# better-flow/better-flow

Hardware: AMD Instinct MI355X
Metric: Mevents/s motion-compensated (warp→converged score), 1M-ev slice, 1/2/4/8 GPU (higher is better)
Workload: dtype f64

## Files before the change

### better_flow_amd/csrc/bf_context.cpp

```cpp
#include "bf_ctx.h"

std::atomic<int> g_live_ctx[64];

extern "C" {

const char* bf_version(void) { return "bf_accel gfx950 r5"; }

int bf_device_count(int32_t* count) {
    int n = 0;
    hipError_t e = hipGetDeviceCount(&n);
    if (count) *count = (e == hipSuccess) ? n : 0;
    return (e == hipSuccess && n > 0) ? BF_OK : BF_ERR_NODEVICE;
}

int bf_abi_struct_sizes(int32_t* out, int32_t n) {
    const int32_t sz[10] = {(int32_t)sizeof(bf_model),     (int32_t)sizeof(bf_window),
                            (int32_t)sizeof(bf_run_opts),  (int32_t)sizeof(bf_run_info),
                            (int32_t)sizeof(bf_trace_rec), (int32_t)sizeof(bf_profile),
                            (int32_t)sizeof(bf_local_window), (int32_t)sizeof(bf_local_state),
                            (int32_t)sizeof(bf_global_pyramid_opts), (int32_t)sizeof(bf_global_pyramid_info)};
    if (!out) return 10;
    const int32_t m = n < 0 ? 0 : (n < 10 ? n : 10);
    for (int i = 0; i < m; ++i) out[i] = sz[i];
    return m;
// ... 140 lines not shown
    }
    delete c;
}

const char* bf_last_error(const bf_ctx* c) {
    if (!c) return "null ctx";
    static thread_local char text[sizeof(c->err)];
    std::lock_guard<std::mutex> g(const_cast<bf_ctx*>(c)->err_mu);
    memcpy(text, c->err, sizeof(text));
    text[sizeof(text) - 1] = 0;
    return text;
}

int bf_get_stat(bf_ctx* c, const char* key, int64_t* value) {
    if (!c || !key || !value) return BF_ERR_ARG;
    if (!strcmp(key, "scatter_format")) {
        *value = c->use_binned ? c->fmt : -1;
        return BF_OK;
    }
    if (!strcmp(key, "one_kernel")) {
        *value = plan_one_kernel(c) ? 1 : 0;
        return BF_OK;
    }
    if (!strcmp(key, "persistent")) {
        *value = plan_persistent(c) ? 1 : 0;
        return BF_OK;
    }
    if (!strcmp(key, "persist_giveups")) {
        *value = c->persist_giveups;
        return BF_OK;
    }
    const struct { const char* name; int v; } launched[] = {
        {"k1_threads", c->launched.k1_threads}, {"k1_events_per_thread", c->launched.k1_per_thread}, {"k1_head", c->launched.k1_head},
        {"k3_half_scale", c->launched.k3_half_scale}, {"k3_mode", c->launched.k3_mode}, {"k3_capped", c->launched.k3_capped},
        {"bin_rows", c->use_binned ? c->grid.TSR : 0}, {"bin_cols", c->use_binned ? c->grid.TS : 0},
        {"bin_margin", c->use_binned ? c->grid.D : 0}, {"bins", c->use_binned ? c->grid.nbins : 0},
        {"groups_lds", c->groups_lds}, {"groups_per_cu", c->groups_per_cu},
        {"propose_form", c->propose_form}};
    for (const auto& e : launched)
        if (!strcmp(key, e.name)) {
            *value = e.v;
            return BF_OK;
        }
    return fail(c, BF_ERR_ARG, "unknown statistic '%s'", key);
}

int bf_set_option(bf_ctx* c, const char* key, int64_t value) {
    if (!c || !key) return BF_ERR_ARG;
    if (!strcmp(key, "force_split")) {
        c->force_split = value != 0;
        return BF_OK;
    }
    if (!strcmp(key, "binned")) {
        if (value < 0 || value > 2) return fail(c, BF_ERR_ARG, "binned must be 0, 1 or 2");
        c->opt_binned = (int)value;
        return BF_OK;
    }
    if (!strcmp(key, "bin_pack_limit")) {
        if (value < 1 || value > 64) return fail(c, BF_ERR_ARG, "bin_pack_limit must be in [1, 64]");
        c->opt_bin_pack_limit = (int)value;
        return BF_OK;
    }
    if (!strcmp(key, "co_schedule")) {
        c->opt_co_schedule = value != 0;
        return BF_OK;
    }
    if (!strcmp(key, "stream_prealloc")) {
        if (!value) return BF_OK;
        HIP_TRY(c, hipSetDevice(c->device));
        const int rc = streaming_setup(c);
        if (rc != BF_OK) return rc;
        for (bf_ctx::UploadSlot& s : c->up.slot) {
            HIP_TRY(c, s.ts.grow((size_t)c->cap_events));
            HIP_TRY(c, s.in16.grow((size_t)c->cap_events * 2));
            HIP_TRY(c, s.noise.grow((size_t)c->cap_events));
        }
        return BF_OK;
    }
    if (!strcmp(key, "sep_update")) {
        if (value < 0 || value > 2) return fail(c, BF_ERR_ARG, "sep_update must be 0 (never), 1 (auto) or 2 (always)");
        c->opt_sep_update = (int)value;
        return BF_OK;
    }
    if (!strcmp(key, "defer_uploads")) {
        if (!value) {
            HIP_TRY(c, hipSetDevice(c->device));
            const int rc = issue_deferred_uploads(c);
            if (rc != BF_OK) return rc;
        }
        c->opt_defer_uploads = value != 0;
        return BF_OK;
    }
    if (!strcmp(key, "watchdog_ms")) {
        if (value < 1) return fail(c, BF_ERR_ARG, "watchdog_ms must be >= 1");
        c->opt_watchdog_s = (double)value * 1e-3;
        return BF_OK;
    }
    if (!strcmp(key, "bin_compact")) {
        if (value < 0 || value > 2) return fail(c, BF_ERR_ARG, "bin_compact must be 0 (never), 1 (auto) or 2 (always)");
        c->opt_bin_compact = (int)value;
        return BF_OK;
    }
    if (!strcmp(key, "bin_split")) {
        if (value < 0 || value > 2) return fail(c, BF_ERR_ARG, "bin_split must be 0, 1 or 2");
        c->opt_bin_split = (int)value;
        return BF_OK;
    }
    if (!strcmp(key, "bin_predict")) {
        c->opt_bin_predict = value != 0;
        return BF_OK;
    }
    if (!strcmp(key, "fused")) {
        if (value < 0 || value > 2) return fail(c, BF_ERR_ARG, "fused must be 0, 1 (auto) or 2");
// ... 188 lines not shown
```

### better_flow_amd/csrc/bf_ctx.h

```cpp
#pragma once
#pragma clang diagnostic ignored "-Wunused-function"
#include <hip/hip_runtime.h>

#include <atomic>
#include <cerrno>
#include <climits>
#include <cmath>
#include <cstdarg>
#include <cstdio>
#include <cstdlib>
#include <chrono>
#include <cstring>
#include <ctime>
#include <memory>
#include <mutex>
#include <new>
#include <utility>
#include <string>
#include <thread>
#include <vector>

#include "bf_assign.h"
#include "bf_device.h"
#include "bf_kernels.h"
// ... 174 lines not shown
    DevArray<uint8_t> d_seg_mask;
    bool seg_valid = false;
    int seg_K = 0;
    SliceStats stats;
    bool stats_valid = false;

    HostArray<DevState> h_state;
    unsigned long long* h_seq = nullptr;
    unsigned long long seq_counter = 0;
    Event poll_ev[2];
    double opt_watchdog_s = 40.0;
    HostArray<SliceStats> h_stats;

    DevState hst;
    bf_window win;
    bool uploaded = false, have_window = false;
    bool has_noise = false, all_noise = false;
    bool packed = true;
    bool force_split = false;
    bool degenerate = false;
    bool pending_warp = false;
    bool n_valid = false;
    uint32_t run_counter = 0;
    int warm_iters_hint = 6;
    bool p_clean = false;
    bool out_sorted = false;
    DevArray<double2> d_out_tmp;
    bool uv_valid = false;
    int cur = 0;
    bool planes_unknown = true;
    int last_R = 0, last_C = 0;

    struct Launched {
        int k1_threads = -1, k1_per_thread = -1, k1_head = -1;
        int k3_half_scale = -1, k3_mode = -1, k3_capped = -1;
    } launched;

    int prof_mode = 0;
    std::vector<ProfRec> prof_pending;
    std::vector<Event> ev_pool;
    bf_profile prof;

    char err[512];
    std::mutex err_mu;
};

extern "C" int ctx_device_uv(bf_ctx* c, const double2** uv);

extern "C" int ctx_device_nxny(bf_ctx* c, const double2** nxny);

struct GlobalHeldFlow {
    const uint32_t* xy; const float2* p; const uint32_t* idx; const double2 *nxny, *uv;
    long long n;
};
int global_held_flow(bf_ctx* c, const char* who, GlobalHeldFlow* out);

struct GlobalBestState {
    const double *max_score, *best_nx, *best_ny;
    long long n;
    double nz;
};
int global_best_state(bf_ctx* c, const bf_global_search_opts* lattice, std::vector<double>& xs, std::vector<double>& ys,
                      GlobalBestState* out);
void global_cand_uv(double nx, double ny, double nz, double* u, double* v);

extern "C" int render_projection_img(bf_ctx* c, int32_t scale, int32_t res_x, int32_t res_y, int32_t show_final, uint8_t* d_img);
extern "C" int render_projection_img_of(bf_ctx* c, const uint32_t* xy, const float2* p, const uint8_t* noise, long long n,
                                        int32_t scale, int32_t res_x, int32_t res_y, int32_t show_final, uint8_t* d_img);
extern "C" int render_color_time_img(bf_ctx* c, int32_t scale, int32_t res_x, int32_t res_y, int32_t show_final, uint8_t* d_bgr);

int ctx_time_img_pass(bf_ctx* c, const char* who);

struct SlicePlan {
    BinGrid grid{}, fgrid{};
    bool binned = false, fused_ok = false, fused_shared = false;
    int fmt = 0, zw = 0;
};
struct RunPlan {
    bool fused = false, binned = false, persist = false;
    bool head_update = false, sep_update = false;
    bool split = false;
    int bin_threads = 0, ev_per_thread = 8;
    bool warm_start = false, prewarp = false, first_warp = false;
    bool quick_warm = false, snap_polled = false;
    double drift_limit = 1e300;
    bool head_like() const { return head_update || sep_update; }
};
SlicePlan plan_slice(const bf_ctx* c, const bf_window& w);
bool plan_one_kernel(const bf_ctx* c);
bool plan_persistent(const bf_ctx* c);
RunPlan plan_run(bf_ctx* c, const bf_run_opts& o);

int streaming_setup(bf_ctx* c);
int issue_deferred_uploads(bf_ctx* c);
void drop_uploads(bf_ctx* c, int k);

namespace {

int fail(bf_ctx* c, int code, const char* fmt, ...) {
    if (c) {
        va_list ap;
        va_start(ap, fmt);
        std::lock_guard<std::mutex> g(c->err_mu);
        vsnprintf(c->err, sizeof(c->err), fmt, ap);
        va_end(ap);
    }
    return code;
}

#define HIP_TRY(c, expr)                                                                      \
    do {                                                                                      \
        hipError_t e__ = (expr);                                                              \
        if (e__ != hipSuccess)                                                                \
            return fail((c), BF_ERR_HIP, "%s failed: %s (%s:%d)", #expr, hipGetErrorString(e__), \
                        __FILE__, __LINE__);                                                  \
    } while (0)

Event get_event(bf_ctx* c) {
    Event e;
// ... 328 lines not shown
```

### better_flow_amd/csrc/bf_device_fns.h

```cpp
#pragma once
#include <hip/hip_runtime.h>
#include <limits.h>

#include "bf_device.h"
#include "bf_kernels.h"
#include "../../include/bf_flow_color.h"
#include <math.h>
#include <math.h>

namespace bf {

__device__ __forceinline__ int trunc_x86(double v) { return bf_double_to_int_x86(v); }

__device__ __forceinline__ int trunc_scatter(double v) { return (v == v) ? __double2int_rz(v) : INT_MIN; }

__device__ __forceinline__ bool valid_px(float p) { return p > 1e-6f; }

__device__ __forceinline__ double div_10000(double x) {
    constexpr double R = 1.0 / 10000.0;
    const double q0 = x * R;
    const double r = fma(-q0, 10000.0, x);
    return fma(r, R, q0);
}
__device__ __forceinline__ float div_127(float x) {
// ... 265 lines not shown
    for (int w = 0; w < W; ++w) {
#pragma unroll
        for (int f = 0; f < 3; ++f) in_[f] += (long long)s_part[f * W + w];
#pragma unroll
        for (int f = 3; f < kSumFields; ++f) d_[f - 3] += __longlong_as_double((long long)s_part[f * W + w]);
    }
    t.n = in_[0]; t.sci = in_[1]; t.scj = in_[2];
    t.sgx = d_[0]; t.sgy = d_[1]; t.sigx = d_[2]; t.sigy = d_[3]; t.sjgx = d_[4]; t.sjgy = d_[5];
    return t;
}
template <int THREADS, bool PACK_INTS = false>
__device__ __forceinline__ Sums block_reduce_sums(const Sums& sm, unsigned long long* s_part ,
                                                  const int tid, const int base_i = 0, const int base_j = 0) {
    block_reduce_publish<THREADS, PACK_INTS>(sm, s_part, tid, base_i, base_j);
    return block_reduce_total<THREADS, PACK_INTS>(s_part, base_i, base_j);
}

struct RcpTab {
    double v[kRcpTab];
    constexpr RcpTab() : v{} {
        for (int i = 1; i < kRcpTab; ++i) v[i] = 1.0 / (double)i;
    }
};
static __constant__ RcpTab c_rcp = RcpTab();

__device__ __forceinline__ float time_from_sums(uint32_t cnt, long long tsum_biased, long long tmin, const double* rcp = nullptr) {
    if (cnt == 0) return 0.f;
    const long long ts = tsum_biased + (long long)(int)cnt * (long long)(int)tmin;
    const float sum_s = (float)div_1e9((double)ts);
    if (rcp && cnt < (uint32_t)kRcpTab) return (float)((double)sum_s * rcp[cnt]);
    return sum_s / (float)cnt;
}

__device__ __attribute__((noinline)) static void sincos_large(double x, double* sn, double* cs) { sincos(x, sn, cs); }
__device__ __forceinline__ void sincos_small(double x, double* sn, double* cs) {
    if (!(fabs(x) <= 0.25)) {
        sincos_large(x, sn, cs);
        return;
    }
    const double z = x * x;
    double ps = -1.0 / 1307674368000.0;
    ps = fma(ps, z, 1.0 / 6227020800.0);
    ps = fma(ps, z, -1.0 / 39916800.0);
    ps = fma(ps, z, 1.0 / 362880.0);
    ps = fma(ps, z, -1.0 / 5040.0);
    ps = fma(ps, z, 1.0 / 120.0);
    ps = fma(ps, z, -1.0 / 6.0);
    *sn = fma(x * z, ps, x);
    double pc = 1.0 / 20922789888000.0;
    pc = fma(pc, z, -1.0 / 87178291200.0);
    pc = fma(pc, z, 1.0 / 479001600.0);
    pc = fma(pc, z, -1.0 / 3628800.0);
    pc = fma(pc, z, 1.0 / 40320.0);
    pc = fma(pc, z, -1.0 / 720.0);
    pc = fma(pc, z, 1.0 / 24.0);
    *cs = 1.0 - z * fma(-z, pc, 0.5);
}

__device__ __forceinline__ void sincos_table_fill(double* tab) {
    tab[0] = -1.0 / 1307674368000.0; tab[1] = 1.0 / 6227020800.0; tab[2] = -1.0 / 39916800.0; tab[3] = 1.0 / 362880.0;
    tab[4] = -1.0 / 5040.0; tab[5] = 1.0 / 120.0; tab[6] = -1.0 / 6.0;
    tab[7] = 1.0 / 20922789888000.0; tab[8] = -1.0 / 87178291200.0; tab[9] = 1.0 / 479001600.0; tab[10] = -1.0 / 3628800.0;
    tab[11] = 1.0 / 40320.0; tab[12] = -1.0 / 720.0; tab[13] = 1.0 / 24.0;
}
__device__ __forceinline__ void sincos_small_tab(double x, const double* tab, double* sn, double* cs) {
    if (!(fabs(x) <= 0.25)) {
        sincos_large(x, sn, cs);
        return;
    }
    const double z = x * x;
    double c_[14];
#pragma unroll
    for (int i = 0; i < 14; ++i) c_[i] = tab[i];
    double ps = c_[0];
    ps = fma(ps, z, c_[1]);
    ps = fma(ps, z, c_[2]);
    ps = fma(ps, z, c_[3]);
    ps = fma(ps, z, c_[4]);
    ps = fma(ps, z, c_[5]);
    ps = fma(ps, z, c_[6]);
    *sn = fma(x * z, ps, x);
    double pc = c_[7];
    pc = fma(pc, z, c_[8]);
    pc = fma(pc, z, c_[9]);
    pc = fma(pc, z, c_[10]);
    pc = fma(pc, z, c_[11]);
    pc = fma(pc, z, c_[12]);
    pc = fma(pc, z, c_[13]);
    *cs = 1.0 - z * fma(-z, pc, 0.5);
}

__device__ __forceinline__ double lane_f64(double v, int lane) {
    const long long b = __double_as_longlong(v);
    const unsigned int lo = (unsigned int)__builtin_amdgcn_readlane((int)(unsigned int)b, lane);
    const unsigned int hi = (unsigned int)__builtin_amdgcn_readlane((int)(unsigned int)((unsigned long long)b >> 32), lane);
    return __longlong_as_double((long long)(((unsigned long long)hi << 32) | (unsigned long long)lo));
}
__device__ __forceinline__ long long lane_i64(unsigned long long v, int lane) {
    const unsigned int lo = (unsigned int)__builtin_amdgcn_readlane((int)(unsigned int)v, lane);
    const unsigned int hi = (unsigned int)__builtin_amdgcn_readlane((int)(unsigned int)(v >> 32), lane);
// ... 396 lines not shown
```

### better_flow_amd/csrc/bf_kernels.h

```cpp
#pragma once
#include <hip/hip_runtime.h>
#include <hip/hip_ext.h>
#include <stdint.h>
#include <atomic>

#include "bf_device.h"
#include "bf_plan_rules.h"

namespace bf {

constexpr int kHistCopies = 8;
using bf_rules::kBinTileLdsMax;
static_assert(bf_rules::kStencilTileR == kTileR && bf_rules::kStencilTileC == kTileC, "the rules count the stencil kernel's own tiles");
constexpr int kPrepBlocks = 1024;

struct SliceStats {
    int32_t xmin, xmax, ymin, ymax, tmin, tmax;
    long long tsum;
};

struct WarpScatterArgs {
    const uint32_t* xy;
    const int32_t* t;
    float2* p;
// ... 126 lines not shown
void launch_fill_states(DevState* states, const DevState& tmpl, int nt, hipStream_t s);
constexpr int kGroupLdsBudget = 156 * 1024;
int launch_group_sort(const uint32_t* xy, const int32_t* t, const uint32_t* perm_in, long long n, const int32_t* gid, int K,
                      uint32_t* hist, uint32_t* start, uint32_t* cursor, uint32_t* oxy, int32_t* ot, float2* op,
                      uint32_t* operm, hipStream_t s);
void launch_group_boxes(const uint32_t* xy, const uint32_t* perm, const int32_t* gid, const uint32_t* start, long long n, int K,
                        int32_t* box, hipStream_t s);
int launch_group_optimizer(const TileArgs& a, const uint32_t* order, int K, bool warm, uint32_t* counter, int n_cus,
                           hipStream_t s, int* per_cu_out);
void launch_group_rest(const uint32_t* perm, const uint32_t* start, int K, double2* nxny, hipStream_t s);

int bin_kernel_setup();
void launch_stencil_binned(const StencilArgs& a, dim3 grid, hipStream_t s, int n_cus);
void launch_margin_clean(unsigned long long* mplane, const uint32_t* mlist, uint32_t* mcount, int nbins, int mcap, hipStream_t s);
void launch_rebin(const EvSets& sets, int has_perm, long long n, DevState* st, const BinGrid& g,
                  uint16_t* binid, uint32_t* hist_cnt, uint32_t* bin_start,
                  uint32_t* cursor, uint32_t* armed, const WarpParams* prewarp, int pack_limit, hipStream_t s,
                  uint32_t* ftab = nullptr, uint32_t* lost = nullptr);
struct BinScatterArgs {
    EvSets sets;
    const uint32_t* bin_start;
    unsigned long long* slabs;
    uint16_t* cidx;
    uint32_t* chdr;
    int compact;
    unsigned long long* ovf_plane;
    uint32_t* ovf_cplane;
    uint32_t* ovf_bits;
    int ovf_pitch;
    const DevState* st_in;
    DevState* st_out;
    DevState* snap;
    MomentAcc* acc;
    uint32_t* ovf_cur;
    const uint32_t* ovf_prev;
    bf_trace_rec* trace;
    BinGrid g;
    int cur, j;
    unsigned long long* tl;
    unsigned long long* m_cur;
    unsigned long long* m_prev;
    uint32_t* mlist;
    uint32_t* mcount;
    int mcap;
};
hipError_t launch_bin_warp_scatter(const BinScatterArgs& a, bool warp, int threads, int per_thread, hipStream_t s);
struct FusedArgs {
    EvSets sets;
    const uint32_t* ftab;
    const DevState* st_in;
    DevState* st_out;
    DevState* snap;
    MomentAcc* acc_in;
    MomentAcc* acc_out;
    MomentAcc* acc_zero;
    uint32_t* lost;
    bf_trace_rec* trace;
    int nbr, nbc;
    int R, C;
    int j;
    int warp;
    unsigned long long* tl;
};
hipError_t launch_fused_pass(const FusedArgs& a, int half_scale, int rows_per_tile, hipStream_t s);
struct FusedLoopArgs {
    EvSets sets;
// ... 188 lines not shown
```

### better_flow_amd/csrc/bf_plan.cpp

```cpp
#include "bf_ctx.h"

SlicePlan plan_slice(const bf_ctx* c, const bf_window& w) {
    SlicePlan p;
    const int scale = w.scale;
    BinGrid& g = p.grid;
    const int bin_margin = bf_rules::bin_margin(c->dbg_margin);
    const bf_rules::BinShape shape = bf_rules::bin_shape(c->n, w.scale_img_x, w.scale_img_y, c->n_cus, bin_margin);
    g.TS = shape.TS;
    g.TSR = shape.TSR;
    g.lg = 0;
    while ((1 << g.lg) < g.TS) ++g.lg;
    g.nbc = shape.nbc;
    g.D = shape.D;
    g.L = g.TS + 2 * g.D;
    g.LR = g.TSR + 2 * g.D;
    g.mul_r = (uint32_t)(0x100000000ull / (unsigned)g.TSR) + 1u;
    g.mul_l = (uint32_t)(0x100000000ull / (unsigned)g.L) + 1u;
    g.mul_h = (uint32_t)(0x100000000ull / (unsigned)(g.L / 2 > 0 ? g.L / 2 : 1)) + 1u;
    g.nbr = shape.nbr;
    g.nbins = shape.nbins;
    const bool dense = (double)w.scale_img_x * (double)w.scale_img_y < 12.0 * (double)c->n ||
                       (double)w.scale_img_x * (double)w.scale_img_y <= 9.0e6;
    p.binned = (c->opt_binned == 2 || (c->opt_binned == 1 && dense)) && !c->force_split && !c->has_noise && c->n > 0 &&
               c->cap_events < (1ll << 29) &&
// ... 23 lines not shown
    const bool lists_ok = p.binned && bf_rules::bin_format_ok(shape, 2);
    const int mode = lists_ok ? c->opt_bin_compact : 0;
    if (mode == 2 || (mode == 1 && 4.0 * (double)c->n < Pimg)) p.fmt = 2;
    const bool split_pays = !c->opt_co_schedule && Pimg >= 1.5e6;
    if (p.fmt == 0 && p.binned && (c->opt_bin_split == 2 || (c->opt_bin_split == 1 && split_pays)) &&
        bf_rules::bin_format_ok(shape, 3))
        p.fmt = 3;
    if (p.fmt == 2 && g.TS == 64 && g.L >= 2 * (g.D + scale / 2 + 1)) p.zw = g.D + scale / 2 + 1;
    return p;
}

bool plan_one_kernel(const bf_ctx* c) {
    return c->fused_ok && (!c->opt_co_schedule || c->fused_shared);
}

bool plan_persistent(const bf_ctx* c) {
    return plan_one_kernel(c) && !c->opt_co_schedule && (c->opt_persist == 2 || (c->opt_persist == 1 && c->pending_warp)) &&
           g_live_ctx[c->device & 63].load() == 1 &&
           fused_loop_resident(c->win.scale / 2, c->fgrid.TSR, c->n_cus, c->fgrid.nbr * c->fgrid.nbc);
}

RunPlan plan_run(bf_ctx* c, const bf_run_opts& o) {
    RunPlan p;
    p.fused = plan_one_kernel(c);
    p.binned = c->use_binned || p.fused;
    p.persist = plan_persistent(c);
    if (p.persist && c->persist_skip > 0) { --c->persist_skip; p.persist = false; }
    p.warm_start = c->pending_warp;
    p.prewarp = p.binned && c->pending_warp;
    p.first_warp = c->pending_warp && !p.prewarp;
    if (p.binned) p.drift_limit = c->opt_bin_predict ? (p.persist ? 0.85 : 0.6) * (double)(p.fused ? c->fgrid.D : c->grid.D) : 1e300;
    p.split = c->use_binned && !p.fused && c->fmt == 3;
    p.head_update = p.fused || (p.binned && !c->opt_co_schedule);
    p.sep_update = p.binned && !p.fused && !p.head_update && (c->opt_sep_update == 2 || (c->opt_sep_update == 1 && c->fmt == 2));
    if (p.binned) {
        const bf_rules::ScatterSize k1 = bf_rules::scatter_size(c->fmt, p.head_update, c->grid.nbins, c->n, c->n_cus);
        p.bin_threads = k1.threads;
        p.ev_per_thread = k1.per_thread;
    }
    p.quick_warm = p.warm_start && c->warm_iters_hint < 3 * o.poll_interval;
    p.snap_polled = p.binned && !p.quick_warm;
    return p;
}
```

### better_flow_amd/csrc/bf_run.cpp

```cpp
#include "bf_ctx.h"

namespace {

struct HostTiming {
#ifdef BF_DEBUG_HOOKS
    bool on = [] { static const bool e = getenv("BF_HOST_TIMING") != nullptr; return e; }();
#else
    static constexpr bool on = false;
#endif
    double launch = 0, wait = 0, mark = on ? now() : 0;
    static double now() { return std::chrono::duration<double>(std::chrono::steady_clock::now().time_since_epoch()).count(); }
    void lap(double& into) { if (on) { const double t = now(); into += t - mark; mark = t; } }
};

struct RunLoop {
    bf_ctx* c;
    const RunPlan& p;
    int b0 = 0, buf = 0;
    bool first = true;
    int launched_iters = 0;
    bool prewarp_done = false;
    bf_trace_rec* trace = nullptr;
    bool want_rebin = false;
    int last_rebin_at = 0;
// ... 155 lines not shown
        FusedArgs fa;
        fa.sets = ev_sets(c);
        fa.ftab = c->d_ftab;
        fa.st_in = L.state_of(j); fa.st_out = L.state_of(j + 1);
        fa.snap = snap;
        fa.acc_in = L.acc_of(j - 1); fa.acc_out = L.acc_of(j); fa.acc_zero = L.acc_of(j + 1);
        fa.lost = lost_flag(c);
        fa.trace = L.trace;
        fa.nbr = c->fgrid.nbr; fa.nbc = c->fgrid.nbc;
        fa.R = c->win.scale_img_x; fa.C = c->win.scale_img_y;
        fa.j = j;
        fa.warp = warp ? 1 : 0;
        fa.tl = c->d_tl;
        ProfScope ps(c, 0, c->n);
        HIP_TRY(c, launch_fused_pass(fa, c->win.scale / 2, c->fgrid.TSR, c->stream));
        L.inf.launches += 1;
    } else {
        const int buf = L.buf;
        if (p.sep_update) {
            launch_finish_update(L.state_of(j), L.acc_of(j - 1), L.ovf_of(j - 1), j, buf ^ 1, L.trace, snap, c->stream);
            L.inf.launches++;
        }
        if (p.binned) {
            BinScatterArgs ba;
            ba.sets = ev_sets(c);
            ba.bin_start = c->d_bin_start;
            ba.slabs = c->d_slabs;
            ba.cidx = c->d_cidx; ba.chdr = c->d_chdr;
            ba.compact = c->fmt;
            ba.ovf_plane = c->d_plane[buf]; ba.ovf_cplane = c->d_cplane[buf];
            ba.ovf_bits = c->d_ovf_bits[buf]; ba.ovf_pitch = c->ovf_pitch;
            ba.st_in = L.state_of(j); ba.st_out = L.state_of(j + 1);
            ba.acc = p.head_update ? L.acc_of(j - 1) : nullptr;
            ba.ovf_cur = L.ovf_of(j); ba.ovf_prev = L.ovf_of(j - 1);
            ba.snap = snap;
            ba.trace = L.trace;
            ba.g = c->grid;
            ba.cur = buf; ba.j = j;
            ba.tl = c->d_tl ? c->d_tl + 64 * 2 * 16 : nullptr;
            ba.m_cur = c->d_mplane[buf]; ba.m_prev = c->d_mplane[buf ^ 1];
            ba.mlist = c->d_mlist; ba.mcount = c->d_mcount; ba.mcap = c->m_cap;
            ProfScope ps(c, 0, c->n);
            HIP_TRY(c, launch_bin_warp_scatter(ba, warp, p.bin_threads, p.ev_per_thread, c->stream));
            c->launched.k1_threads = p.bin_threads; c->launched.k1_per_thread = p.ev_per_thread; c->launched.k1_head = p.head_update ? 1 : 0;
        } else {
            ProfScope ps(c, 0, c->n);
            launch_warp_scatter(ws_args(c, buf, 1), warp, true, false, c->stream);
        }
        StencilArgs a = st_args(c, buf, 1);
        if (p.binned) {
            a.ovf_bits = c->d_ovf_bits[buf]; a.zero_bits = c->d_ovf_bits[buf ^ 1]; a.ovf_pitch = c->ovf_pitch;
            a.zero_full = j == 0 ? 1 : 0;
            a.st = L.state_of(j + 1);
            a.ovf_cur = L.ovf_of(j); a.ovf_prev = L.ovf_of(j - 1); a.ovf_next = L.ovf_of(j + 1);
            a.tile_bands = (!p.head_update && c->fmt != 2) ? 1 : 0;
        }
        if (p.head_like()) {
            a.acc = L.acc_of(j); a.acc_zero = L.acc_of(j + 1);
        } else if (p.binned) {
            a.acc = c->d_acc;
            a.ticket = c->d_ticket;
            a.st = L.state_of(j);
            a.st_rw = L.state_of(j + 1);
            a.snap = snap;
        } else {
            a.acc = c->d_acc;
            a.ticket = c->d_ticket;
            a.st_rw = c->d_state;
        }
        a.trace = L.trace;
        a.update_mode = 1;
        a.tl = c->d_tl;
        a.tl_launch = j;
        ProfScope ps(c, 1);
        const bool shared_lists = c->opt_co_schedule && c->fmt == 2 && g_live_ctx[c->device & 63].load() > 1;
        const int k3_cus = shared_lists ? 1 : c->n_cus;
        launch_stencil(a, stencil_src(c, p.binned), c->stream, k3_cus);
// ... 273 lines not shown
```

### better_flow_amd/csrc/bf_scatter.hip

```cpp
#include <atomic>
#include <hip/hip_runtime.h>
#include <hip/hip_ext.h>
#include <limits.h>
#include <cstdlib>

#include "bf_device.h"
#include "bf_device_fns.h"
#include "bf_kernels.h"

namespace bf {

template <class T>
__device__ __forceinline__ T ld_idx(const T* base, uint32_t idx) {
    return *reinterpret_cast<const T*>(reinterpret_cast<const char*>(base) + idx * (uint32_t)sizeof(T));
}

constexpr int kMaxTileRows = 192;

struct ScatterGeo {
    int X0, Y0, L, LR;
    int zw;
};
template <bool WARP>
__device__ __forceinline__ bool event_target(const ScatterHot& hs, float2* p, uint32_t i, uint32_t v, int32_t ti,
// ... 313 lines not shown
                    if (cd != kNoEntry) list_put(hs, sg, a, s_row, cd, r, vt[k], (uint32_t)LL, vals, cidx, n_ovf);
                }
            }
        }
        if (n_ovf) { atomicAdd(ovf_counter(a.ovf_cur, b), n_ovf); a.ovf_cur[0] = 1u; }
        tl_stamp(a.tl, a.j, 4);
        return;
    }
    for (;;) {
#pragma unroll
        for (int k = 0; k < U; ++k) {
            const uint32_t i = base + k * THREADS + tid;
            if (i >= end) continue;
            scatter_event<WARP>(hs, sg, s_tile, a, p, i, vxy[k], vt[k], ppx[k], ppy[k], n_ovf);
        }
        base += THREADS * U;
        if (base >= end) break;
        load_pass();
        previous_positions();
    }
    if (n_ovf) { atomicAdd(ovf_counter(a.ovf_cur, b), n_ovf); a.ovf_cur[0] = 1u; }
    if (SPLIT) margin_clear(a, b, m_prev_n, m_e0, tid, THREADS);
    tl_stamp(a.tl, a.j, 2);
    __syncthreads();
    tl_stamp(a.tl, a.j, 3);
    store_state();
    if (SPLIT) flush_split<THREADS>(s_tile, a, b, X0, Y0, hs.C, s_mcnt, tid);
    else flush_tile<THREADS>(s_tile, a.slabs + (size_t)b * (size_t)LL, LL, tid);
    tl_stamp(a.tl, a.j, 4);
}

template <bool WARP, int THREADS, int U, int FMT>
__global__ __launch_bounds__(THREADS) void k_bin_warp_scatter_lean(const uint32_t* __restrict__ pre_bin_start, const DevState* pre_st_in,
                                                                   MomentAcc* , BinScatterArgs a) {
    constexpr bool COMPACT = FMT == 2;
    constexpr bool SPLIT = FMT == 3;
    extern __shared__ unsigned long long s_tile[];
    __shared__ uint32_t s_row[FMT == 2 ? 1 + 3 * kMaxTileRows : 1];
    __shared__ uint32_t s_mcnt[2];
    if (FMT == 2)
        for (int r = threadIdx.x; r <= 3 * kMaxTileRows; r += THREADS) s_row[r] = 0;
    if (SPLIT && threadIdx.x < 2) s_mcnt[threadIdx.x] = 0;
    const BinGrid& g = a.g;
    const int L = g.L, LR = g.LR, LL = g.LR * g.L;
    const int b = blockIdx.x, tid = threadIdx.x;
    const uint32_t beg = sload(pre_bin_start + b), end = sload(pre_bin_start + b + 1);
    const HotState h0 = sload(&pre_st_in->hot);
    const uint32_t m_prev_n = SPLIT ? sload(a.mcount + b) : 0u;
    const int X0 = (b / g.nbc) * g.TSR - g.D, Y0 = (b - (b / g.nbc) * g.nbc) * g.TS - g.D;
    if (!COMPACT) {
        ulonglong2* z = reinterpret_cast<ulonglong2*>(s_tile);
        for (int i = tid; i < LL / 2; i += THREADS) z[i] = make_ulonglong2(0ull, 0ull);
    }
    if (h0.done) {
        if (b == 0 && tid < kStateWords) {
            const unsigned long long state_word = reinterpret_cast<const unsigned long long*>(a.st_in)[tid];
            reinterpret_cast<unsigned long long*>(a.st_out)[tid] = state_word;
            if (a.snap) reinterpret_cast<unsigned long long*>(a.snap)[tid] = state_word;
        }
        return;
    }
    ScatterHot hs;
    hs.done = h0.done; hs.bin_tbits = h0.bin_tbits; hs.bin_ok = h0.bin_ok; hs.fmt = h0.fmt; hs.scale = h0.scale; hs.C = h0.C;
    hs.wsx = h0.wsx; hs.wsy = h0.wsy; hs.x_sh = h0.x_sh; hs.y_sh = h0.y_sh; hs.tmin = h0.tmin; hs.wp = h0.wp;
    const EvSetPtrs ev = a.sets.s[h0.cs ^ h0.flip];
    const uint32_t* __restrict__ xy = ev.xy;
    const int32_t* __restrict__ t = ev.t;
    float2* __restrict__ p = ev.p;
    const ScatterGeo sg = {X0, Y0, L, LR, FMT == 2 ? g.zw : 0};
    uint32_t n_ovf = 0;
    __syncthreads();
    uint32_t vxy[U];
    int32_t vt[U];
    float2 vp[U];
    auto load_pass = [&](uint32_t base) {
#pragma unroll
        for (int k = 0; k < U; ++k) {
            uint32_t i = base + k * THREADS + tid;
            i = i < end ? i : beg;
            vxy[k] = ld_idx(xy, i);
            vt[k] = ld_idx(t, i);
            vp[k] = ld_idx(p, i);
        }
    };
    if constexpr (COMPACT) {
        const bool single = end - beg <= (uint32_t)(THREADS * U);
// ... 31 lines not shown
                    if (i >= end) continue;
                    int r;
                    const uint32_t cd = list_event<false>(hs, sg, a, p, i, vxy[k], vt[k], pr_from_p(vxy[k] & 0xffffu, vp[k].x),
                                                          pr_from_p(vxy[k] >> 16, vp[k].y), false, r, n_ovf);
                    if (cd != kNoEntry) list_put(hs, sg, a, s_row, cd, r, vt[k], (uint32_t)LL, vals, cidx, n_ovf);
                }
            }
        }
        if (n_ovf) { atomicAdd(ovf_counter(a.ovf_cur, b), n_ovf); a.ovf_cur[0] = 1u; }
        return;
    }
    auto scatter_pass = [&](uint32_t base) {
#pragma unroll
        for (int k = 0; k < U; ++k) {
            const uint32_t i = base + k * THREADS + tid;
            if (i >= end) continue;
            scatter_event<WARP>(hs, sg, s_tile, a, p, i, vxy[k], vt[k], pr_from_p(vxy[k] & 0xffffu, vp[k].x),
                                pr_from_p(vxy[k] >> 16, vp[k].y), n_ovf);
        }
    };
    if constexpr (SPLIT) {
        const uint32_t m_e0 = margin_preload(a, b, m_prev_n, tid);
        uint32_t base = beg;
        load_pass(base);
        for (;;) {
            scatter_pass(base);
            base += THREADS * U;
            if (base >= end) break;
            load_pass(base);
        }
        if (n_ovf) { atomicAdd(ovf_counter(a.ovf_cur, b), n_ovf); a.ovf_cur[0] = 1u; }
        margin_clear(a, b, m_prev_n, m_e0, tid, THREADS);
    } else {
        for (uint32_t base = beg; base < end; base += THREADS * U) {
            load_pass(base);
            scatter_pass(base);
        }
        if (n_ovf) { atomicAdd(ovf_counter(a.ovf_cur, b), n_ovf); a.ovf_cur[0] = 1u; }
    }
    __syncthreads();
    if (SPLIT) flush_split<THREADS>(s_tile, a, b, X0, Y0, hs.C, s_mcnt, tid);
    else flush_tile<THREADS>(s_tile, a.slabs + (size_t)b * (size_t)LL, LL, tid);
}

__global__ __launch_bounds__(64) void k_finish_update(DevState* st, MomentAcc* acc, const uint32_t* ovf_prev, int j,
                                                            int cur_prev, bf_trace_rec* trace, DevState* snap, const uint32_t* lost,
                                                            unsigned long long* snap_seq, unsigned long long seq) {
    __shared__ DevState s_state;
    const int tid = threadIdx.x;
    const int done = st->hot.done, it = st->hot.it;
    const bool trip = lost && *lost != 0u && st->hot.need_rebin != 2;
    const bool apply = lost ? st->hot.pend != 0 : it < j;
    if (tid < kStateWords)
        reinterpret_cast<unsigned long long*>(&s_state)[tid] = reinterpret_cast<const unsigned long long*>(st)[tid];
    if (trip && !done) {
        __builtin_amdgcn_wave_barrier();
        if (tid == 0) { s_state.hot.need_rebin = 2; s_state.hot.redo = 1; s_state.hot.pend = 0; }
        __builtin_amdgcn_wave_barrier();
        if (tid < kStateWords)
            reinterpret_cast<unsigned long long*>(st)[tid] = reinterpret_cast<const unsigned long long*>(&s_state)[tid];
    } else if (!done && apply) {
        const uint32_t ovf = ovf_total_wave(ovf_part(ovf_prev, tid));
        unsigned long long accv[kAccPerLane];
        acc_load_wave<false, false>(acc, tid, accv);
        const unsigned long long word = acc_reduce_wave(accv);
        __builtin_amdgcn_wave_barrier();
        model_update_wave(&s_state, word, tid, 1);
        if (tid == 0) {
            model_update_rest(&s_state, trace, cur_prev, ovf);
            s_state.hot.pend = 0;
        }
        __builtin_amdgcn_wave_barrier();
        if (tid < kStateWords)
            reinterpret_cast<unsigned long long*>(st)[tid] = reinterpret_cast<const unsigned long long*>(&s_state)[tid];
    }
    if (snap && tid < kStateWords)
        reinterpret_cast<unsigned long long*>(snap)[tid] = reinterpret_cast<const unsigned long long*>(&s_state)[tid];
    if (snap_seq) {
        __threadfence_system();
        if (tid == 0) __hip_atomic_store(snap_seq, seq, __ATOMIC_RELEASE, __HIP_MEMORY_SCOPE_SYSTEM);
    }
}

template <bool HEAD, int THREADS, int U, int FMT>
static hipError_t launch_bws2(const BinScatterArgs& a, bool warp, hipStream_t s) {
    const size_t lds = FMT == 2 ? 0 : (size_t)a.g.LR * a.g.L * sizeof(unsigned long long) + 16;
    static std::atomic<unsigned long long> raised{0ull};
    const void* fns[2] = {HEAD ? reinterpret_cast<const void*>(&k_bin_warp_scatter<true, THREADS, U, FMT>)
                               : reinterpret_cast<const void*>(&k_bin_warp_scatter_lean<true, THREADS, U, FMT>),
                          HEAD ? reinterpret_cast<const void*>(&k_bin_warp_scatter<false, THREADS, U, FMT>)
                               : reinterpret_cast<const void*>(&k_bin_warp_scatter_lean<false, THREADS, U, FMT>)};
    const hipError_t e = raise_dynamic_lds(raised, fns);
    if (e != hipSuccess) return e;
    if constexpr (HEAD) {
        if (warp) launch_timed(k_bin_warp_scatter<true, THREADS, U, FMT>, dim3(a.g.nbins), dim3(THREADS), lds, s, a.bin_start, a.st_in, a.acc, a);
        else launch_timed(k_bin_warp_scatter<false, THREADS, U, FMT>, dim3(a.g.nbins), dim3(THREADS), lds, s, a.bin_start, a.st_in, a.acc, a);
    } else {
        if (warp) launch_timed(k_bin_warp_scatter_lean<true, THREADS, U, FMT>, dim3(a.g.nbins), dim3(THREADS), lds, s, a.bin_start, a.st_in, a.acc, a);
        else launch_timed(k_bin_warp_scatter_lean<false, THREADS, U, FMT>, dim3(a.g.nbins), dim3(THREADS), lds, s, a.bin_start, a.st_in, a.acc, a);
    }
    return hipSuccess;
}
template <bool HEAD, int THREADS, int FMT>
static hipError_t launch_bws(const BinScatterArgs& a, bool warp, int per_thread, hipStream_t s) {
    constexpr bool kWide = THREADS == 1024;
    constexpr bool kEight = FMT == 2 ? THREADS == 512 : (kWide || !HEAD);
    switch (per_thread) {
        case 1: if constexpr (!kWide) return launch_bws2<HEAD, THREADS, 1, FMT>(a, warp, s); else break;
        case 2: return launch_bws2<HEAD, THREADS, 2, FMT>(a, warp, s);
        case 4: return launch_bws2<HEAD, THREADS, 4, FMT>(a, warp, s);
        case 8: if constexpr (kEight) return launch_bws2<HEAD, THREADS, 8, FMT>(a, warp, s); else break;
        case 10: if constexpr (FMT == 0 && !HEAD) return launch_bws2<HEAD, THREADS, 10, FMT>(a, warp, s); else break;
        case 12: if constexpr (FMT == 0 && !HEAD) return launch_bws2<HEAD, THREADS, 12, FMT>(a, warp, s); else break;
        default: break;
    }
    return hipErrorInvalidValue;
}

hipError_t launch_bin_warp_scatter(const BinScatterArgs& a, bool warp, int threads, int per_thread, hipStream_t s) {
    const bool head = a.acc != nullptr;
    if (!bf_rules::scatter_compiled(head, threads, per_thread, a.compact)) return hipErrorInvalidValue;
    if (a.compact == 2) {
        if (threads == 256) return head ? launch_bws<true, 256, 2>(a, warp, per_thread, s) : launch_bws<false, 256, 2>(a, warp, per_thread, s);
        return head ? launch_bws<true, 512, 2>(a, warp, per_thread, s) : launch_bws<false, 512, 2>(a, warp, per_thread, s);
    }
    if (a.compact == 3) {
        if (threads == 1024) return launch_bws<true, 1024, 3>(a, warp, per_thread, s);
        return head ? launch_bws<true, 512, 3>(a, warp, per_thread, s) : launch_bws<false, 512, 3>(a, warp, per_thread, s);
    }
    if (threads == 1024) return launch_bws<true, 1024, 0>(a, warp, per_thread, s);
    return head ? launch_bws<true, 512, 0>(a, warp, per_thread, s) : launch_bws<false, 512, 0>(a, warp, per_thread, s);
}


void launch_finish_update(DevState* st, MomentAcc* acc, const uint32_t* ovf_prev, int j, int cur_prev, bf_trace_rec* trace,
                          DevState* snap, hipStream_t s, const uint32_t* lost, unsigned long long* snap_seq, unsigned long long seq) {
    hipLaunchKernelGGL(k_finish_update, dim3(1), dim3(64), 0, s, st, acc, ovf_prev, j, cur_prev, trace, snap, lost, snap_seq, seq);
}

}
```

Baseline: 212.4.

## Fold the model update into the lean scatter kernel's first wave

Adds a wave-update mode for the uncompressed binned scatter kernel. In every block, the first wavefront reduces the previous iteration's moment accumulator and applies the model update into LDS at raised priority. Meanwhile the other waves prefetch their first batch of events, then spin on an LDS ready flag before scattering with the updated warp parameters. This aims to remove the separate update step and the kernel boundary between update and scatter, at the cost of every block repeating the update and one wave per block doing less scatter work. It also returns sincos_large's result as a double2 instead of through pointers.

```diff
diff --git a/better_flow_amd/csrc/bf_context.cpp b/better_flow_amd/csrc/bf_context.cpp
--- a/better_flow_amd/csrc/bf_context.cpp
+++ b/better_flow_amd/csrc/bf_context.cpp
@@ -196,6 +196,7 @@
     }
     const struct { const char* name; int v; } launched[] = {
         {"k1_threads", c->launched.k1_threads}, {"k1_events_per_thread", c->launched.k1_per_thread}, {"k1_head", c->launched.k1_head},
+        {"k1_wave_update", c->launched.k1_wave_update},
         {"k3_half_scale", c->launched.k3_half_scale}, {"k3_mode", c->launched.k3_mode}, {"k3_capped", c->launched.k3_capped},
         {"bin_rows", c->use_binned ? c->grid.TSR : 0}, {"bin_cols", c->use_binned ? c->grid.TS : 0},
         {"bin_margin", c->use_binned ? c->grid.D : 0}, {"bins", c->use_binned ? c->grid.nbins : 0},
@@ -242,7 +243,8 @@
         return BF_OK;
     }
     if (!strcmp(key, "sep_update")) {
-        if (value < 0 || value > 2) return fail(c, BF_ERR_ARG, "sep_update must be 0 (never), 1 (auto) or 2 (always)");
+        if (value < 0 || value > 3)
+            return fail(c, BF_ERR_ARG, "sep_update must be 0 (never), 1 (auto), 2 (always) or 3 (in the scatter kernel's first waves)");
         c->opt_sep_update = (int)value;
         return BF_OK;
     }
diff --git a/better_flow_amd/csrc/bf_ctx.h b/better_flow_amd/csrc/bf_ctx.h
--- a/better_flow_amd/csrc/bf_ctx.h
+++ b/better_flow_amd/csrc/bf_ctx.h
@@ -230,7 +230,7 @@
     int last_R = 0, last_C = 0;
 
     struct Launched {
-        int k1_threads = -1, k1_per_thread = -1, k1_head = -1;
+        int k1_threads = -1, k1_per_thread = -1, k1_head = -1, k1_wave_update = -1;
         int k3_half_scale = -1, k3_mode = -1, k3_capped = -1;
     } launched;
 
@@ -277,12 +277,13 @@
 struct RunPlan {
     bool fused = false, binned = false, persist = false;
     bool head_update = false, sep_update = false;
+    bool wave_update = false;
     bool split = false;
     int bin_threads = 0, ev_per_thread = 8;
     bool warm_start = false, prewarp = false, first_warp = false;
     bool quick_warm = false, snap_polled = false;
     double drift_limit = 1e300;
-    bool head_like() const { return head_update || sep_update; }
+    bool head_like() const { return head_update || sep_update || wave_update; }
 };
 SlicePlan plan_slice(const bf_ctx* c, const bf_window& w);
 bool plan_one_kernel(const bf_ctx* c);
diff --git a/better_flow_amd/csrc/bf_device_fns.h b/better_flow_amd/csrc/bf_device_fns.h
--- a/better_flow_amd/csrc/bf_device_fns.h
+++ b/better_flow_amd/csrc/bf_device_fns.h
@@ -321,10 +321,16 @@
     return sum_s / (float)cnt;
 }
 
-__device__ __attribute__((noinline)) static void sincos_large(double x, double* sn, double* cs) { sincos(x, sn, cs); }
+__device__ __attribute__((noinline)) static double2 sincos_large(double x) {
+    double2 r;
+    sincos(x, &r.x, &r.y);
+    return r;
+}
 __device__ __forceinline__ void sincos_small(double x, double* sn, double* cs) {
     if (!(fabs(x) <= 0.25)) {
-        sincos_large(x, sn, cs);
+        const double2 r = sincos_large(x);
+        *sn = r.x;
+        *cs = r.y;
         return;
     }
     const double z = x * x;
@@ -354,7 +360,9 @@
 }
 __device__ __forceinline__ void sincos_small_tab(double x, const double* tab, double* sn, double* cs) {
     if (!(fabs(x) <= 0.25)) {
-        sincos_large(x, sn, cs);
+        const double2 r = sincos_large(x);
+        *sn = r.x;
+        *cs = r.y;
         return;
     }
     const double z = x * x;
diff --git a/better_flow_amd/csrc/bf_kernels.h b/better_flow_amd/csrc/bf_kernels.h
--- a/better_flow_amd/csrc/bf_kernels.h
+++ b/better_flow_amd/csrc/bf_kernels.h
@@ -182,6 +182,8 @@
     DevState* st_out;
     DevState* snap;
     MomentAcc* acc;
+    int wave_update;
+    MomentAcc* wave_acc;
     uint32_t* ovf_cur;
     const uint32_t* ovf_prev;
     bf_trace_rec* trace;
diff --git a/better_flow_amd/csrc/bf_plan.cpp b/better_flow_amd/csrc/bf_plan.cpp
--- a/better_flow_amd/csrc/bf_plan.cpp
+++ b/better_flow_amd/csrc/bf_plan.cpp
@@ -79,7 +79,7 @@
     if (p.binned) p.drift_limit = c->opt_bin_predict ? (p.persist ? 0.85 : 0.6) * (double)(p.fused ? c->fgrid.D : c->grid.D) : 1e300;
     p.split = c->use_binned && !p.fused && c->fmt == 3;
     p.head_update = p.fused || (p.binned && !c->opt_co_schedule);
-    p.sep_update = p.binned && !p.fused && !p.head_update && (c->opt_sep_update == 2 || (c->opt_sep_update == 1 && c->fmt == 2));
+    p.sep_update = p.binned && !p.fused && !p.head_update && (c->opt_sep_update == 2 || ((c->opt_sep_update == 1 || c->opt_sep_update == 3) && c->fmt == 2));
     if (p.binned) {
         const bf_rules::ScatterSize k1 = bf_rules::scatter_size(c->fmt, p.head_update, c->grid.nbins, c->n, c->n_cus);
         p.bin_threads = k1.threads;
@@ -87,5 +87,6 @@
     }
     p.quick_warm = p.warm_start && c->warm_iters_hint < 3 * o.poll_interval;
     p.snap_polled = p.binned && !p.quick_warm;
+    p.wave_update = (c->opt_sep_update == 3 || c->opt_sep_update == 1) && p.binned && !p.fused && !p.head_update && !p.sep_update && c->fmt == 0 && !p.quick_warm;
     return p;
 }
diff --git a/better_flow_amd/csrc/bf_run.cpp b/better_flow_amd/csrc/bf_run.cpp
--- a/better_flow_amd/csrc/bf_run.cpp
+++ b/better_flow_amd/csrc/bf_run.cpp
@@ -211,6 +211,8 @@
             ba.ovf_bits = c->d_ovf_bits[buf]; ba.ovf_pitch = c->ovf_pitch;
             ba.st_in = L.state_of(j); ba.st_out = L.state_of(j + 1);
             ba.acc = p.head_update ? L.acc_of(j - 1) : nullptr;
+            ba.wave_update = p.wave_update ? 1 : 0;
+            ba.wave_acc = p.wave_update ? L.acc_of(j - 1) : nullptr;
             ba.ovf_cur = L.ovf_of(j); ba.ovf_prev = L.ovf_of(j - 1);
             ba.snap = snap;
             ba.trace = L.trace;
@@ -222,6 +224,7 @@
             ProfScope ps(c, 0, c->n);
             HIP_TRY(c, launch_bin_warp_scatter(ba, warp, p.bin_threads, p.ev_per_thread, c->stream));
             c->launched.k1_threads = p.bin_threads; c->launched.k1_per_thread = p.ev_per_thread; c->launched.k1_head = p.head_update ? 1 : 0;
+            c->launched.k1_wave_update = p.wave_update ? 1 : 0;
         } else {
             ProfScope ps(c, 0, c->n);
             launch_warp_scatter(ws_args(c, buf, 1), warp, true, false, c->stream);
diff --git a/better_flow_amd/csrc/bf_scatter.hip b/better_flow_amd/csrc/bf_scatter.hip
--- a/better_flow_amd/csrc/bf_scatter.hip
+++ b/better_flow_amd/csrc/bf_scatter.hip
@@ -369,7 +369,10 @@
 
 template <bool WARP, int THREADS, int U, int FMT>
 __global__ __launch_bounds__(THREADS) void k_bin_warp_scatter_lean(const uint32_t* __restrict__ pre_bin_start, const DevState* pre_st_in,
-                                                                   MomentAcc* , BinScatterArgs a) {
+                                                                   MomentAcc* pre_acc ,
+                                                                   BinScatterArgs a) {
+    constexpr bool WAVE_UPD = FMT == 0;
+    __shared__ unsigned long long s_wu[WAVE_UPD ? kStateWords + 1 : 1];
     constexpr bool COMPACT = FMT == 2;
     constexpr bool SPLIT = FMT == 3;
     extern __shared__ unsigned long long s_tile[];
@@ -381,6 +384,16 @@
     const BinGrid& g = a.g;
     const int L = g.L, LR = g.LR, LL = g.LR * g.L;
     const int b = blockIdx.x, tid = threadIdx.x;
+    const bool wave_upd = WAVE_UPD && pre_acc != nullptr;
+    const bool first_wave = __builtin_amdgcn_readfirstlane(tid >> 6) == 0;
+    unsigned long long accv[kAccPerLane];
+    unsigned long long state_word = 0;
+    uint32_t ovf_prev_part = 0;
+    if (WAVE_UPD && wave_upd && first_wave) {
+        acc_load_wave<false, false>(pre_acc, tid, accv);
+        if (b == 0) ovf_prev_part = ovf_part(a.ovf_prev, tid);
+        if (tid < kStateWords) state_word = reinterpret_cast<const unsigned long long*>(pre_st_in)[tid];
+    }
     const uint32_t beg = sload(pre_bin_start + b), end = sload(pre_bin_start + b + 1);
     const HotState h0 = sload(&pre_st_in->hot);
     const uint32_t m_prev_n = SPLIT ? sload(a.mcount + b) : 0u;
@@ -389,6 +402,7 @@
         ulonglong2* z = reinterpret_cast<ulonglong2*>(s_tile);
         for (int i = tid; i < LL / 2; i += THREADS) z[i] = make_ulonglong2(0ull, 0ull);
     }
+    if (WAVE_UPD && wave_upd && tid == 0) s_wu[kStateWords] = 0ull;
     if (h0.done) {
         if (b == 0 && tid < kStateWords) {
             const unsigned long long state_word = reinterpret_cast<const unsigned long long*>(a.st_in)[tid];
@@ -486,13 +500,83 @@
         if (n_ovf) { atomicAdd(ovf_counter(a.ovf_cur, b), n_ovf); a.ovf_cur[0] = 1u; }
         margin_clear(a, b, m_prev_n, m_e0, tid, THREADS);
     } else {
-        for (uint32_t base = beg; base < end; base += THREADS * U) {
+        uint32_t base0 = beg;
+        if (WAVE_UPD && wave_upd) {
+            DevState* const sst = reinterpret_cast<DevState*>(s_wu);
+            uint32_t* const s_ready = reinterpret_cast<uint32_t*>(s_wu + kStateWords);
+            const bool pending = h0.it < a.j;
+            static_assert(THREADS > 64, "the first wave updates, the others take the first pass");
+            constexpr int T1 = THREADS - 64;
+            const int t1 = tid - 64;
+            if (first_wave) {
+                if (tid < kStateWords) s_wu[tid] = state_word;
+                if (pending) {
+                    __builtin_amdgcn_s_setprio(3);
+                    const unsigned long long word = acc_reduce_wave(accv);
+                    __builtin_amdgcn_wave_barrier();
+                    model_update_wave(sst, word, tid, 1);
+                    __builtin_amdgcn_wave_barrier();
+                    if (tid == 0) __hip_atomic_store(s_ready, 1u, __ATOMIC_RELEASE, __HIP_MEMORY_SCOPE_WORKGROUP);
+                    __builtin_amdgcn_s_setprio(0);
+                    if (b == 0) {
+                        const uint32_t ovf_prev = ovf_total_wave(ovf_prev_part);
+                        if (tid == 0) model_update_rest(sst, a.trace, a.cur ^ 1, ovf_prev);
+                    }
+                }
+            } else {
+                if (beg < end) {
+#pragma unroll
+                    for (int k = 0; k < U; ++k) {
+                        uint32_t i = beg + k * T1 + t1;
+                        i = i < end ? i : beg;
+                        vxy[k] = ld_idx(xy, i);
+                        vt[k] = ld_idx(t, i);
+                        vp[k] = ld_idx(p, i);
+                    }
+                }
+                asm volatile("" ::: "memory");
+                if (pending)
+                    while (__hip_atomic_load(s_ready, __ATOMIC_ACQUIRE, __HIP_MEMORY_SCOPE_WORKGROUP) == 0u) __builtin_amdgcn_s_sleep(1);
+            }
+            if (pending) {
+                __builtin_amdgcn_wave_barrier();
+                hs.wp = lds_uniform(&sst->hot.wp);
+                hs.done = lds_sreg(&sst->hot.done);
+            }
+            if (hs.done) {
+                if (b == 0 && first_wave) {
+                    __builtin_amdgcn_wave_barrier();
+                    if (tid < kStateWords) {
+                        const unsigned long long v = s_wu[tid];
+                        reinterpret_cast<unsigned long long*>(a.st_out)[tid] = v;
+                        if (a.snap) reinterpret_cast<unsigned long long*>(a.snap)[tid] = v;
+                    }
+                }
+                return;
+            }
+            if (!first_wave && beg < end) {
+#pragma unroll
+                for (int k = 0; k < U; ++k) {
+                    const uint32_t i = beg + k * T1 + t1;
+                    if (i >= end) continue;
+                    scatter_event<WARP>(hs, sg, s_tile, a, p, i, vxy[k], vt[k], pr_from_p(vxy[k] & 0xffffu, vp[k].x),
+                                        pr_from_p(vxy[k] >> 16, vp[k].y), n_ovf);
+                }
+            }
+            base0 = beg + (uint32_t)(T1 * U);
+        }
+        for (uint32_t base = base0; base < end; base += THREADS * U) {
             load_pass(base);
             scatter_pass(base);
         }
         if (n_ovf) { atomicAdd(ovf_counter(a.ovf_cur, b), n_ovf); a.ovf_cur[0] = 1u; }
     }
     __syncthreads();
+    if (WAVE_UPD && wave_upd && b == 0 && tid < kStateWords) {
+        const unsigned long long v = s_wu[tid];
+        reinterpret_cast<unsigned long long*>(a.st_out)[tid] = v;
+        if (a.snap) reinterpret_cast<unsigned long long*>(a.snap)[tid] = v;
+    }
     if (SPLIT) flush_split<THREADS>(s_tile, a, b, X0, Y0, hs.C, s_mcnt, tid);
     else flush_tile<THREADS>(s_tile, a.slabs + (size_t)b * (size_t)LL, LL, tid);
 }
@@ -550,8 +634,8 @@
         if (warp) launch_timed(k_bin_warp_scatter<true, THREADS, U, FMT>, dim3(a.g.nbins), dim3(THREADS), lds, s, a.bin_start, a.st_in, a.acc, a);
         else launch_timed(k_bin_warp_scatter<false, THREADS, U, FMT>, dim3(a.g.nbins), dim3(THREADS), lds, s, a.bin_start, a.st_in, a.acc, a);
     } else {
-        if (warp) launch_timed(k_bin_warp_scatter_lean<true, THREADS, U, FMT>, dim3(a.g.nbins), dim3(THREADS), lds, s, a.bin_start, a.st_in, a.acc, a);
-        else launch_timed(k_bin_warp_scatter_lean<false, THREADS, U, FMT>, dim3(a.g.nbins), dim3(THREADS), lds, s, a.bin_start, a.st_in, a.acc, a);
+        if (warp) launch_timed(k_bin_warp_scatter_lean<true, THREADS, U, FMT>, dim3(a.g.nbins), dim3(THREADS), lds, s, a.bin_start, a.st_in, a.wave_acc, a);
+        else launch_timed(k_bin_warp_scatter_lean<false, THREADS, U, FMT>, dim3(a.g.nbins), dim3(THREADS), lds, s, a.bin_start, a.st_in, a.wave_acc, a);
     }
     return hipSuccess;
 }
@@ -574,6 +658,7 @@
 hipError_t launch_bin_warp_scatter(const BinScatterArgs& a, bool warp, int threads, int per_thread, hipStream_t s) {
     const bool head = a.acc != nullptr;
     if (!bf_rules::scatter_compiled(head, threads, per_thread, a.compact)) return hipErrorInvalidValue;
+    if ((a.wave_update != 0) != (a.wave_acc != nullptr) || (a.wave_update && (head || a.compact != 0))) return hipErrorInvalidValue;
     if (a.compact == 2) {
         if (threads == 256) return head ? launch_bws<true, 256, 2>(a, warp, per_thread, s) : launch_bws<false, 256, 2>(a, warp, per_thread, s);
         return head ? launch_bws<true, 512, 2>(a, warp, per_thread, s) : launch_bws<false, 512, 2>(a, warp, per_thread, s);
```

New measurement: 215.3 (median of 5 runs). 1.01x the previous value.
